# wang-xinyu/tensorrtx

Measured on AMD Instinct MI355X. Metric: images/sec @ batch=32 640x640 fp16 (yolov8n conv backbone + YoloLayer decode + NMS), higher is better.
Workload: dtype f16

## Files before the change

include/trtx_hip.h:

```cpp
#ifndef TRTX_HIP_H_
#define TRTX_HIP_H_

#include <stddef.h>
#include <stdint.h>

#ifdef __cplusplus
extern "C" {
#endif

#ifndef TRTX_NO_HIP_TYPES
struct ihipStream_t;
typedef struct ihipStream_t* trtx_stream_t;
#endif

#define TRTX_ABI_VERSION 1
#define TRTX_OK 0
#define TRTX_ERR_INVALID 1
#define TRTX_ERR_HIP 2
#define TRTX_ERR_WORKSPACE 3
#define TRTX_ERR_UNSUPPORTED 4
#define TRTX_ERR_NO_DEVICE 5
#define TRTX_ERR_IO 6
#define TRTX_ERR_STATE 7

// ... 138 lines not shown
#define TRTX_ACT_TANH 5
int32_t trtx_conv_packed_dims(int cout, int cin_pad, int kh, int kw, int32_t* cout_pad, int32_t* kpad, int32_t* bn);
int32_t trtx_conv_pack_weights_f16(const float* w_kcrs, int cout, int cin, int kh, int kw, int cin_pad,
                                   const float* ch_scale, uint16_t* packed);
int32_t trtx_op_conv2d_nhwc_f16(const void* in, int N, int H, int W, int Cin, int ld_in, const void* wpacked,
                                const float* bias, void* out, int Cout, int ld_out, int kh, int kw, int sh, int sw,
                                int ph, int pw, int act1, const void* residual, int ld_res, int act2,
                                trtx_stream_t stream);
int32_t trtx_op_conv2d_tactics(int N, int H, int W, int Cin, int ld_in, int Cout, int ld_out, int kh, int kw, int sh, int sw, int ph, int pw,
                               int has_residual, int ld_res, int32_t* out6, int32_t max_out);
int32_t trtx_op_conv_force_tactic(const int32_t* tactic6);
int32_t trtx_op_conv_stem_nchw_f16(const float* in, int N, int C, int H, int W, const float* w_taps_cout, const float* bias, void* out, int Cout,
                                   int ld_out, int k, int stride, int pad, int act, trtx_stream_t stream);
int32_t trtx_op_conv_stem_pair_f16(const float* in, int N, int C, int H, int W, const float* stem_w_taps_cout, const float* stem_bias, int stem_act,
                                   const void* conv_wpacked, const float* conv_bias, int conv_act, void* out, int ld_out, trtx_stream_t stream);
int32_t trtx_reorg_fold_weights(const float* w_kcrs, int cout, int cin, int kh, int kw, float* folded);
int32_t trtx_conv_packed_dims_f32(int cout, int cin_pad, int kh, int kw, int32_t* cout_pad, int32_t* kpad, int32_t* cink);
int32_t trtx_conv_pack_weights_f32(const float* w_kcrs, int cout, int cin, int kh, int kw, int cin_pad, const float* ch_scale, float* packed);
int32_t trtx_op_conv2d_nhwc_f32(const void* in, int N, int H, int W, int Cin, int ld_in, const void* wpacked, const float* bias, void* out, int Cout,
                                int ld_out, int kh, int kw, int sh, int sw, int ph, int pw, int act1, const void* residual, int ld_res, int act2,
                                const int32_t* tile4, trtx_stream_t stream);
int32_t trtx_op_conv2d_tactics_f32(int N, int H, int W, int Cin, int ld_in, int Cout, int ld_out, int kh, int kw, int sh, int sw, int ph, int pw,
                                   int has_residual, int ld_res, int32_t* out4, int32_t max_out);
int32_t trtx_conv_pack_weights_i8(const float* w_kcrs, int cout, int cin, int kh, int kw, const float* ch_scale, int8_t* packed, float* wscale_out,
                                  int32_t* cout_pad_out, int32_t* kpad_out);
int32_t trtx_op_conv2d_nhwc_i8(const void* in, int N, int H, int W, int Cin, int ld_in, const void* wpacked, const float* cscale, const float* bias, void* out,
                               int out_is_i8, float out_inv_scale, int Cout, int ld_out, int kh, int kw, int sh, int sw, int ph, int pw, int act1,
                               const void* residual, int res_is_i8, float res_scale, int ld_res, int act2, trtx_stream_t stream);
int32_t trtx_conv_pack_weights_grouped_f16(const float* w_kcrs, int cout, int cin_g, int kh, int kw, const float* ch_scale, uint16_t* packed,
                                           int32_t* kpad_out);
// ... 225 lines not shown
```

tensorrtx_amd/capi.py:

```python
import ctypes
import os

_HERE = os.path.dirname(os.path.abspath(__file__))
_LIB = None


class TrtxError(RuntimeError):
    def __init__(self, status, what):
        self.status = status
        msg = lib().trtx_status_string(status).decode() if _LIB is not None else "?"
        super().__init__(f"{what}: status {status} ({msg})")


def lib_path() -> str:
    return os.environ.get("TRTX_HIP_LIB") or os.path.join(_HERE, "lib", "libtrtx_hip.so")


def hip_runtimes_mapped():
    seen = []
    with open("/proc/self/maps") as f:
        for line in f:
            path = line.rsplit(" ", 1)[-1].strip()
            if "libamdhip64" in os.path.basename(path) and path not in seen:
                seen.append(path)
# ... 442 lines not shown
    return out


def conv_stem_pair_f16(x, stem_w_taps_cout, stem_bias, conv_wpacked, conv_bias, stem_act="silu", conv_act="silu", out=None, out_ld=None):
    import torch
    N, C, H, W = x.shape
    Hi, Wi = (H - 1) // 2 + 1, (W - 1) // 2 + 1
    Ho, Wo = (Hi - 1) // 2 + 1, (Wi - 1) // 2 + 1
    if out is None:
        out = torch.empty((N, Ho, Wo, 32), dtype=torch.float16, device=x.device)
    check(lib().trtx_op_conv_stem_pair_f16(_p(x), N, C, H, W, _p(stem_w_taps_cout), _p(stem_bias), ACT[stem_act], _p(conv_wpacked), _p(conv_bias),
                                           ACT[conv_act], _p(out), out_ld or out.shape[-1], _stream()), "trtx_op_conv_stem_pair_f16")
    return out


def pack_conv_weights_grouped_f16(w_kcrs, ch_scale=None):
    import numpy as np
    L = lib()
    w = np.ascontiguousarray(w_kcrs, dtype=np.float32)
    cout, cin_g, kh, kw = w.shape
    kp = ctypes.c_int32()
    check(L.trtx_conv_pack_weights_grouped_f16(w.ctypes.data_as(ctypes.c_void_p), cout, cin_g, kh, kw, None, None, ctypes.byref(kp)),
          "trtx_conv_pack_weights_grouped_f16 (dims)")
    packed = np.zeros((cout, kp.value), dtype=np.uint16)
    sc = None if ch_scale is None else np.ascontiguousarray(ch_scale, dtype=np.float32)
    check(L.trtx_conv_pack_weights_grouped_f16(w.ctypes.data_as(ctypes.c_void_p), cout, cin_g, kh, kw,
                                               sc.ctypes.data_as(ctypes.c_void_p) if sc is not None else None,
                                               packed.ctypes.data_as(ctypes.c_void_p), ctypes.byref(kp)), "trtx_conv_pack_weights_grouped_f16")
    return packed

# ... 200 lines not shown
```

tensorrtx_amd/csrc/kernels/kernels.h:

```cpp
#pragma once
#include <hip/hip_runtime.h>
#include <stddef.h>
#include <stdint.h>

namespace trtx {

enum Act : int { ACT_NONE = 0, ACT_RELU = 1, ACT_SIGMOID = 2, ACT_SILU = 3, ACT_LEAKY = 4, ACT_TANH = 5,
                 ACT_MISH = 6 ,
                 ACT_GELU_TANH = 7 ,
                 ACT_EXP = 8  };
enum DType : int { DT_F32 = 0, DT_F16 = 1, DT_I8 = 2 };
inline size_t dtype_size(int dt) { return dt == DT_F16 ? 2 : (dt == DT_I8 ? 1 : 4); }
enum EwOp : int { EW_SUM = 0, EW_PROD = 1, EW_MAX = 2, EW_MIN = 3, EW_SUB = 4, EW_DIV = 5, EW_POW = 6 };
enum PoolOp : int { POOL_MAX = 0, POOL_AVG = 1 };

enum Ws : int {
    WS_AUTO = 0,
    WS_OFF = 1,
    WS_ON = 2,
    WS_PATCH = 3,
    WS_F32_REGS = 5,
    WS_F32_ROLES = 6,
    WS_RES3 = 7,
    WS_RES1 = 8,
// ... 74 lines not shown
int32_t conv_ws_f16(const ConvArgs& a, hipStream_t s);
int32_t poison_lds(unsigned* device_word, hipStream_t s);
bool conv_stem_supported(const ConvArgs& a);
int32_t conv_stem_nchw_f32(const ConvArgs& a, hipStream_t s);
bool conv_stem_f32_supported(const ConvArgs& a);
int32_t conv_stem_nchw_f32_out_f32(const ConvArgs& a, hipStream_t s);
constexpr int kStemMaxFrames = 64;
struct StemFrame {
    const void* src;
    int w, h;
    float d2s[6];
};
int32_t conv_stem_frames_f32(const ConvArgs& a, const StemFrame* frames, hipStream_t s);
bool conv_stem_pair_possible(const ConvArgs& stem, const ConvArgs& conv);
int32_t conv_stem_pair_f16(const ConvArgs& stem, const ConvArgs& conv, hipStream_t s);
int32_t conv_direct(const ConvArgs& a, int dtype, hipStream_t s);
bool conv_dw_supported(const ConvArgs& a);
bool psa_attention_supported(int kd, int hd);
int32_t psa_attention_f16(const void* qkv, int ld_qkv, void* out, int ld_out, void* vimg, int ld_v, int B, int heads, int N, int kd, int hd,
                          float scale, hipStream_t s);
bool area_attention_supported(int kd, int hd);
int32_t area_attention_f16(const void* qkv, int ld_qkv, void* out, int ld_out, void* vimg, int ld_v, int B, int heads, int N, int area, int kd,
                           int hd, float scale, hipStream_t s);
bool area_attention_split_supported(int kd, int hd);
int32_t area_attention_split_f16(const void* q, int ld_q, const void* k, int ld_k, const void* v, int ld_v, void* out, int ld_out, int B, int heads, int N,
                                 int area, int kd, int hd, float scale, hipStream_t s);
int32_t conv_dw(const ConvArgs& a, int dtype, hipStream_t s);
struct HgconvWeights {
    const float* w_ctx;
    const float* b_ctx;
// ... 67 lines not shown
```

tensorrtx_amd/csrc/ops_capi.cpp:

```cpp
#include <hip/hip_runtime.h>
#include <stdlib.h>
#include <string.h>

#include <vector>

#include "common.h"
#include "options.h"
#include "kernels/kernels.h"
#include "runtime/pack.h"

using namespace trtx;

extern "C" const char* trtx_status_string(int32_t s) {
    switch (s) {
        case TRTX_OK: return "ok";
        case TRTX_ERR_INVALID: return "invalid argument";
        case TRTX_ERR_HIP: return "HIP error";
        case TRTX_ERR_WORKSPACE: return "workspace too small";
        case TRTX_ERR_UNSUPPORTED: return "unsupported configuration";
        case TRTX_ERR_NO_DEVICE: return "no HIP device";
        case TRTX_ERR_IO: return "I/O or parse error";
        case TRTX_ERR_STATE: return "invalid call order";
        default: return "unknown status";
    }
// ... 120 lines not shown
    a.ld_out = ld_out;
    return conv_stem_nchw_f32(a, static_cast<hipStream_t>(stream));
}

extern "C" int32_t trtx_op_conv_stem_pair_f16(const float* in, int N, int C, int H, int W, const float* stem_w_taps_cout, const float* stem_bias, int stem_act,
                                              const void* conv_wpacked, const float* conv_bias, int conv_act, void* out, int ld_out, trtx_stream_t stream) {
    if (!in || !stem_w_taps_cout || !conv_wpacked || !out || N < 1 || C < 1 || H < 1 || W < 1) return TRTX_ERR_INVALID;
    const ConvArgs s = op_stem_args(in, N, C, H, W, stem_w_taps_cout, stem_bias, 16, 3, 2, 1, stem_act);
    ConvArgs c = op_conv_args(N, s.Ho, s.Wo, 16, 16, 32, ld_out, 3, 3, 2, 2, 1, 1, conv_act, 0, 0, 0);
    c.wgt = conv_wpacked;
    c.bias = conv_bias;
    c.out = out;
    return conv_stem_pair_f16(s, c, static_cast<hipStream_t>(stream));
}

extern "C" int32_t trtx_conv_pack_weights_grouped_f16(const float* w_kcrs, int cout, int cin_g, int kh, int kw, const float* ch_scale, uint16_t* packed,
                                                      int32_t* kpad_out) {
    if (!w_kcrs || cout < 1 || cin_g < 1 || kh < 1 || kw < 1) return TRTX_ERR_INVALID;
    const int kpad = (kh * kw * cin_g + 31) / 32 * 32;
    if (kpad_out) *kpad_out = kpad;
    if (packed) pack_conv_weights_grouped_f16(w_kcrs, cout, cin_g, kh, kw, kpad, ch_scale, packed);
    return TRTX_OK;
}

extern "C" int32_t trtx_op_conv2d_grouped_nhwc_f16(const void* in, int N, int H, int W, int Cin, int ld_in, const void* wpacked, const float* bias, void* out,
                                                   int Cout, int ld_out, int groups, int k, int pad, int act1, const void* residual, int ld_res, int act2,
                                                   trtx_stream_t stream) {
    if (N < 1 || H < 1 || W < 1 || Cin < 1 || Cout < 1 || groups < 1 || k < 1 || pad < 0 || H + 2 * pad < k || W + 2 * pad < k) return TRTX_ERR_INVALID;
    ConvArgs a{};
    a.in = in; a.wgt = wpacked; a.bias = bias; a.out = out; a.residual = residual;
// ... 210 lines not shown
```

tensorrtx_amd/csrc/options.cpp:

```cpp
#include "options.h"

#include <stdlib.h>

namespace trtx {
namespace {
const char* env(const char* name) { return getenv(name); }
int env_int(const char* name, int unset) {
    const char* v = env(name);
    return (v && *v) ? atoi(v) : unset;
}
bool env_is(const char* name, int value) {
    const char* v = env(name);
    return v && *v && atoi(v) == value;
}
bool env_set(const char* name) { return env(name) != nullptr; }
}

Options read_options() {
    Options o;
    o.tune = env_int("TRTX_TUNE", -1);
    o.tune_verbose = env_set("TRTX_TUNE_VERBOSE");
    o.tune_margin = env_int("TRTX_TUNE_MARGIN", -1);
    if (const char* v = env("TRTX_TACTIC_CACHE")) o.tactic_cache = v;
    o.graph = env_is("TRTX_GRAPH", 1);
    if (const char* v = env("TRTX_CALIB_REPORT")) o.calib_report = v;
    if (const char* v = env("TRTX_INT8_CLIP_LIMIT"); v && *v) o.int8_clip_limit = atof(v);
    o.lanes = env_int("TRTX_LANES", 0);
    o.group_convs = !env_is("TRTX_GROUP_CONVS", 0);
    o.fold_upsample = !env_is("TRTX_FOLD_UPSAMPLE", 0);
    o.stem_pair = !env_is("TRTX_STEM_PAIR", 0);
    o.ws = !env_set("TRTX_CONV_NOWS");
    o.wsk = !env_set("TRTX_CONV_NOWSK");
    o.gemm256 = !env_is("TRTX_GEMM256", 0);
    o.patch = !env_is("TRTX_CONV_PATCH", 0);
    o.res = env_int("TRTX_CONV_RES", 7);
    o.roles = !env_is("TRTX_CONV_ROLES", 0);
    o.f32_mfma = !env_set("TRTX_F32_DIRECT");
    o.conv_grouped = !env_is("TRTX_CONV_GROUPED", 0);
    o.area_attention = !env_is("TRTX_AREA_ATTENTION", 0);
    o.aattn_split = !env_is("TRTX_AATTN_SPLIT", 0);
    o.hgconv = !env_is("TRTX_HGCONV", 0);
    o.gated_add = !env_is("TRTX_GATED_ADD", 0);
    o.yolo5_head = !env_is("TRTX_YOLO5_HEAD", 0);
    o.yolo7_head = !env_is("TRTX_YOLO7_HEAD", 0);
    o.reorg_fold = !env_is("TRTX_REORG_FOLD", 0);
// ... 16 lines not shown
```

tensorrtx_amd/csrc/options.h:

```cpp
#pragma once
#include <string>

namespace trtx {

struct Options {
    int tune = -1;
    bool tune_verbose = false;
    int tune_margin = -1;
    std::string tactic_cache;
    bool graph = false;
    std::string calib_report;
    double int8_clip_limit = 1e-4;
    int lanes = 0;
    bool group_convs = true;
    bool fold_upsample = true;
    bool stem_pair = true;
    bool ws = true;
    bool wsk = true;
    bool gemm256 = true;
    bool patch = true;
    int res = 7;
    bool roles = true;
    bool f32_mfma = true;
    bool conv_grouped = true;
    bool area_attention = true;
    bool aattn_split = true;
    bool hgconv = true;
    bool gated_add = true;
    bool yolo9_head = true;
    bool yolo5_head = true;
    bool yolo7_head = true;
// ... 13 lines not shown
```

tensorrtx_amd/csrc/runtime/engine.cpp:

```cpp
#include "engine.h"

#include <stdlib.h>
#include <string.h>

#include <sstream>

#include "../common.h"
#include "../options.h"
#include "int8.h"
#include "plugin.h"

using namespace trtx;

trtx_engine::~trtx_engine() {
    int left = plugins_initialized;
    for (auto& op : plan.ops)
        if (op.kind == OP_PLUGIN && left-- > 0 && op.plugin->v.terminate) op.plugin->v.terminate(op.plugin->v.self);
    if (d_weights) (void)hipFree(d_weights);
}

trtx_context::~trtx_context() {
    for (hipStream_t st : lane_stream)
        if (st) {
            (void)hipStreamSynchronize(st);
// ... 92 lines not shown
    std::vector<char> lane_started(plan.num_lanes, 0);
    auto bail = [&](int32_t st) {
        (void)hipGetLastError();
        if (lanes)
            for (int l = 1; l < plan.num_lanes; ++l)
                if (lane_started[l] && hipEventRecord(c->lane_done[l], c->lane_stream[l]) == hipSuccess)
                    (void)hipStreamWaitEvent(user_stream, c->lane_done[l], 0);
        for (auto& ev : evs) (void)hipEventDestroy(ev);
        evs.clear();
        free_probes();
        return st;
    };
    if (lanes && hipEventRecord(c->start_event, user_stream) != hipSuccess) return bail(TRTX_ERR_HIP);
    ConvArgs pair_stem{};
    bool pair_pending = false;
    for (size_t k = 0; k < plan.ops.size(); ++k) {
        const POp& op = plan.ops[k];
        hipStream_t stream = user_stream;
        if (lanes) {
            if (op.lane > 0) {
                stream = c->lane_stream[op.lane];
                if (!lane_started[op.lane]) {
                    if (hipStreamWaitEvent(stream, c->start_event, 0) != hipSuccess) return bail(TRTX_ERR_HIP);
                    lane_started[op.lane] = 1;
                }
            }
            for (int d : op.wait_ops)
                if (hipStreamWaitEvent(stream, c->op_event[d], 0) != hipSuccess) return bail(TRTX_ERR_HIP);
        }
        const PTensor& t0 = plan.tensors[op.in.empty() ? op.out[0] : op.in[0]];
// ... 23 lines not shown
                    b.N = nb(to);
                    b.M = b.N * b.Ho * b.Wo;
                    if (conv_stem_pair_possible(a, b)) {
                        pair_stem = a;
                        pair_pending = true;
                        break;
                    }
                }
                if (op.stem_pair && pair_pending) {
                    pair_pending = false;
                    if (prof && probes[k].start && probes[k].stop) conv_set_launch_probe(&probes[k]);
                    st = conv_stem_pair_f16(pair_stem, a, stream);
                    conv_set_launch_probe(nullptr);
                    break;
                }
                if (op.kind == OP_DECONV)
                    st = deconv_direct(a, op.dtype, stream);
                else if (op.stem && c->frames)
                    st = a.f32 ? TRTX_ERR_UNSUPPORTED : conv_stem_frames_f32(a, c->frames, stream);
                else if (op.stem)
                    st = a.f32 ? conv_stem_nchw_f32_out_f32(a, stream) : conv_stem_nchw_f32(a, stream);
                else if (op.igemm) {
                    if (prof && probes[k].start && probes[k].stop) conv_set_launch_probe(&probes[k]);
                    st = a.f32 ? conv_igemm_f32(a, stream) : conv_igemm_f16(a, stream);
                    conv_set_launch_probe(nullptr);
                } else if (op.dw)
                    st = conv_dw(a, op.dtype, stream);
                else if (op.grouped)
                    st = conv_grouped(a, stream);
                else
// ... 655 lines not shown
```

tensorrtx_amd/csrc/runtime/plan.cpp:

```cpp
#include "plan.h"

#include <sstream>

namespace trtx {

const char* op_kind_name(int k) {
    static const char* n[] = {"conv",     "deconv",    "pool",      "resize",     "ew_nhwc", "act_nhwc", "scale_nhwc",
                              "copy_nhwc", "reduce_hw", "to_nhwc",   "to_linear",  "gather",  "scatter",  "ew_lin",
                              "act_lin",  "scale_lin", "softmax",   "matmul",     "reduce_lin", "plugin", "copy_lin", "yolo_head",
                              "pool_chain", "depth_to_space", "roi_align", "conv_chain", "conv_group", "attention",
                              "yolo_task_head", "yolo5_head", "yolo9_head", "yolo7_head", "hgconv", "gated_add", "attention_split"};
    return (k >= 0 && k <= OP_ATTENTION_SPLIT) ? n[k] : "?";
}

std::string Plan::describe_json() const {
    std::ostringstream o;
    double flops = 0, bytes = 0;
    int n_conv = 0, n_igemm = 0;
    for (const auto& op : ops) {
        flops += op.flops;
        bytes += op.bytes;
        if (op.kind == OP_CONV) {
            ++n_conv;
            n_igemm += op.igemm ? 1 : 0;
        }
        n_conv += (int)op.group.size();
        n_igemm += (int)op.group.size();
    }
    o << "{\"fp16\":" << (fp16 ? "true" : "false") << ",\"max_batch\":" << max_batch << ",\"arena_bytes\":" << arena_bytes
      << ",\"weight_bytes\":" << weight_bytes << ",\"n_lanes\":" << num_lanes << ",\"n_ops\":" << ops.size() << ",\"n_conv\":" << n_conv
      << ",\"n_igemm\":" << n_igemm << ",\"flops_per_sample\":" << flops << ",\"bytes_per_sample\":" << bytes
      << ",\"ops\":[";
    for (size_t k = 0; k < ops.size(); ++k) {
        const POp& op = ops[k];
        o << (k ? "," : "") << "{\"kind\":\"" << op_kind_name(op.kind) << "\",\"name\":\"";
        for (char c : op.name) o << ((c == '"' || c == '\\' || (unsigned char)c < 0x20) ? ' ' : c);
        o << "\",\"flops\":" << op.flops << ",\"bytes\":" << op.bytes;
        auto conv_fields = [&](const POp& op) {
            const ConvArgs& a = op.conv;
            o << ",\"igemm\":" << (op.igemm ? "true" : "false") << ",\"stem\":" << (op.stem ? "true" : "false") << (op.stem_pair ? ",\"stem_pair\":true" : "") << ",\"cin\":" << (a.in_i8 ? 2 * a.Cin : a.Cin) << ",\"cout\":" << a.Cout
              << ",\"k\":[" << a.kh << "," << a.kw << "],\"stride\":[" << a.stride_h << "," << a.stride_w << "],\"hw_in\":["
              << a.H << "," << a.W << "],\"hw_out\":[" << a.Ho << "," << a.Wo << "],\"act1\":" << a.act1
              << ",\"act2\":" << a.act2 << ",\"alpha1\":" << a.alpha1 << ",\"alpha2\":" << a.alpha2 << ",\"up_c\":" << a.up_C << ",\"residual\":" << (op.in.size() > 1 ? "true" : "false")
              << ",\"bn_folded\":" << (op.scale_layer >= 0 ? "true" : "false") << ",\"ld_in\":" << a.ld_in
              << ",\"ld_out\":" << a.ld_out << ",\"i8\":[" << a.in_i8 << "," << a.out_i8 << "," << a.res_i8 << "],\"nmul\":" << (op.stem ? 1 : tensors[op.in[0]].nmul) << ",\"nfix\":"
              << (op.stem ? 0 : tensors[op.in[0]].nfix);
            if (op.dw) o << ",\"dw\":true";
            if (op.grouped) o << ",\"grouped\":true";
            if (op.cout_real) o << ",\"cout_real\":" << op.cout_real;
            if (op.reorg_cin) o << ",\"reorg_cin\":" << op.reorg_cin;
        };
        if (op.kind == OP_CONV || op.kind == OP_DECONV) conv_fields(op);
        if (op.kind == OP_ACT_NHWC || op.kind == OP_ACT_LIN) o << ",\"act\":" << op.i[0];
        if (op.kind == OP_ATTENTION) o << ",\"heads\":" << op.i[0] << ",\"n\":" << op.i[1] << ",\"kd\":" << op.i[2] << ",\"hd\":" << op.i[3];
        if (op.kind == OP_ATTENTION && op.i[4] > 0) o << ",\"area\":" << op.i[4] << ",\"kernel\":\"mfma\"";
// ... 75 lines not shown
```

tensorrtx_amd/csrc/runtime/plan.h:

```cpp
#pragma once
#include <memory>
#include <string>
#include <vector>

#include "../kernels/kernels.h"
#include "graph.h"
#include "plugin.h"

namespace trtx {

enum Layout : int { LAY_LINEAR = 0, LAY_NHWC = 1 };
enum StorageKind : int { ST_ARENA = 0, ST_WEIGHTS = 1, ST_BINDING = 2 };

enum OpKind : int {
    OP_CONV = 0,
    OP_DECONV,
    OP_POOL,
    OP_RESIZE,
    OP_EW_NHWC,
    OP_ACT_NHWC,
    OP_SCALE_NHWC,
    OP_COPY_NHWC,
    OP_REDUCE_HW,
    OP_TO_NHWC,
// ... 56 lines not shown
    int binding = -1;
    int first_use = 1 << 30, last_use = -1;
};
inline size_t align256(size_t v) { return (v + 255) / 256 * 256; }

struct POp {
    int kind = 0;
    std::string name;
    std::vector<int> in, out;
    std::vector<int> extra_in;
    int dtype = DT_F32;
    ConvArgs conv{};
    bool igemm = false;
    bool stem = false;
    bool stem_pair = false;
    bool from_deconv = false;
    bool dw = false;
    bool grouped = false;
    int reorg_cin = 0;
    int cout_real = 0;
    std::vector<POp> group;
    int src_layer = -1;
    int scale_layer = -1;
    size_t w_off = 0, b_off = 0, s_off = 0;
    int i[12] = {0};
    float f[4] = {0};
    std::vector<int> iv;
    std::vector<float> fv;
    StridedView view{};
    long off0 = 0;
// ... 39 lines not shown
```

tensorrtx_amd/csrc/runtime/plan_passes.cpp:

```cpp
#include "plan_passes.h"

#include <algorithm>

namespace trtx {
namespace {

bool fail(std::string* err, const std::string& m) {
    *err = m;
    return false;
}

size_t tensor_bytes(const Plan& plan, const PTensor& t) {
    const size_t es = dtype_size(t.dtype);
    if (t.layout == LAY_NHWC) {
        const size_t n = (t.nfix ? (size_t)t.nfix : (size_t)plan.max_batch) * (size_t)t.nmul;
        return n * t.H * t.W * (size_t)t.Calloc * es;
    }
    return (t.batched ? (size_t)plan.max_batch : 1) * (size_t)t.dims.volume() * es;
}

bool choose_conv_kernel(const Plan& plan, const PassInputs& e, POp& op) {
    ConvArgs& a = op.conv;
    const PTensor& ti = plan.tensors[op.in[0]];
    const PTensor& to = plan.tensors[op.out[0]];
// ... 639 lines not shown
            shared = touches(plan.ops[j]);
            for (const POp& m : plan.ops[j].group) shared = shared || touches(m);
        }
        if (shared) continue;
        ConvArgs a = st.conv, b = cv.conv;
        const PTensor& t_in = plan.tensors[st.in[0]];
        a.N = plan.explicit_batch ? (int)t_in.dims.d[0] : plan.max_batch;
        a.M = a.N * a.Ho * a.Wo;
        b.N = (mid.nfix ? mid.nfix : plan.max_batch) * mid.nmul;
        b.M = b.N * b.Ho * b.Wo;
        if (!conv_stem_pair_possible(a, b)) continue;
        cv.stem_pair = true;
    }
}

void assign_lanes(Plan& plan, const PassInputs& e, const std::vector<std::vector<int>>& deps) {
    const int nops = (int)plan.ops.size();
    int max_lanes = e.max_aux_streams >= 0 ? 1 + e.max_aux_streams : 4;
    if (e.opt.lanes > 0) max_lanes = std::max(1, std::min(16, e.opt.lanes));
    std::vector<int> tail(max_lanes, -1);
    plan.num_lanes = 1;
    for (int k = 0; k < nops; ++k) {
        int lane = -1;
        for (int d : deps[k])
            if (tail[plan.ops[d].lane] == d && (lane < 0 || d > tail[lane])) lane = plan.ops[d].lane;
        if (lane < 0 && deps[k].empty()) lane = 0;
        if (lane < 0) {
            for (int l = 0; l < max_lanes && lane < 0; ++l)
                if (tail[l] < 0) lane = l;
        }
// ... 23 lines not shown
    const int nops = (int)plan.ops.size();
    auto before = [&](int a, int b) { return a == b || anc.has(a, b); };
    std::vector<std::vector<int>> touch(plan.storages.size());
    for (int k = 0; k < nops; ++k) {
        const POp& op = plan.ops[k];
        auto mark = [&](int t) {
            const int st = plan.tensors[t].storage;
            Storage& s = plan.storages[st];
            s.first_use = std::min(s.first_use, k);
            s.last_use = std::max(s.last_use, k);
            if (touch[st].empty() || touch[st].back() != k) touch[st].push_back(k);
        };
        for (int t : op.in) mark(t);
        for (int t : op.extra_in) mark(t);
        for (int t : op.out) mark(t);
    }
    std::vector<std::pair<int, int>> ws_storage;
    for (int k = 0; k < nops; ++k) {
        const int kind = plan.ops[k].kind;
        if ((kind != OP_PLUGIN && kind != OP_YOLO_HEAD && kind != OP_YOLO_TASK_HEAD && kind != OP_YOLO5_HEAD && kind != OP_YOLO9_HEAD && kind != OP_YOLO7_HEAD && kind != OP_HGCONV) || plan.ops[k].ws_bytes == 0) continue;
        Storage s;
        s.kind = ST_ARENA;
        s.bytes = plan.ops[k].ws_bytes;
        s.first_use = s.last_use = k;
        ws_storage.push_back({k, (int)plan.storages.size()});
        plan.storages.push_back(s);
        touch.push_back({k});
    }
    auto ordered = [&](int sa, int sb) {
        for (int x : touch[sa])
// ... 31 lines not shown
    for (auto& w : ws_storage) plan.ops[w.first].ws_off = plan.storages[w.second].offset;
}

}

bool finalize_plan(Plan& plan, const PassInputs& e, std::string* err) {
    resolve_view_geometry(plan);
    fold_upsample(plan, e);
    assign_int8_served(plan, e);
    assign_storages(plan);
    if (!select_conv_kernels(plan, e, err) || !configure_plugins(plan, err)) return false;
    chain_sppf_pools(plan, e);
    chain_spp_parallel_pools(plan, e);
    group_convs(plan, e);
    mark_stem_pair(plan, e);
    const std::vector<std::vector<int>> deps = op_dependencies(plan);
    assign_lanes(plan, e, deps);
    plan_arena(plan, ancestors(plan, deps, true));
    return true;
}

}
```

Before: 38910.

## Fuse consecutive 16-channel 3x3 bottleneck convs into one tiled LDS kernel

```diff
diff --git a/include/trtx_hip.h b/include/trtx_hip.h
--- a/include/trtx_hip.h
+++ b/include/trtx_hip.h
@@ -176,6 +176,12 @@
                                    int ld_out, int k, int stride, int pad, int act, trtx_stream_t stream);
 int32_t trtx_op_conv_stem_pair_f16(const float* in, int N, int C, int H, int W, const float* stem_w_taps_cout, const float* stem_bias, int stem_act,
                                    const void* conv_wpacked, const float* conv_bias, int conv_act, void* out, int ld_out, trtx_stream_t stream);
+int32_t trtx_op_conv_bneck_pair_f16(const void* in, int N, int H, int W, int ld_in, int in_coff, const void* w1_packed, const float* bias1, int act1,
+                                    const void* w2_packed, const float* bias2, int act2, int shortcut, int act_after, void* out, int ld_out,
+                                    trtx_stream_t stream);
+int32_t trtx_op_conv_bneck_pair_or_two_f16(const void* in, int N, int H, int W, int ld_in, int in_coff, const void* w1_packed, const float* bias1, int act1,
+                                           const void* w2_packed, const float* bias2, int act2, int shortcut, int act_after, void* mid, void* out,
+                                           int ld_out, trtx_stream_t stream);
 int32_t trtx_reorg_fold_weights(const float* w_kcrs, int cout, int cin, int kh, int kw, float* folded);
 int32_t trtx_conv_packed_dims_f32(int cout, int cin_pad, int kh, int kw, int32_t* cout_pad, int32_t* kpad, int32_t* cink);
 int32_t trtx_conv_pack_weights_f32(const float* w_kcrs, int cout, int cin, int kh, int kw, int cin_pad, const float* ch_scale, float* packed);
diff --git a/tensorrtx_amd/capi.py b/tensorrtx_amd/capi.py
--- a/tensorrtx_amd/capi.py
+++ b/tensorrtx_amd/capi.py
@@ -480,6 +480,22 @@
     return out
 
 
+def conv_bneck_pair_f16(x, w1_packed, bias1, w2_packed, bias2, act1="silu", act2="silu", shortcut=True, act_after="none", out=None, out_ld=None, in_coff=None,
+                        mid=None):
+    import torch
+    N, H, W, C = x.shape
+    assert x.dtype == torch.float16 and x.stride(3) == 1 and (C == 16 if in_coff is None else in_coff + 16 <= C)
+    if out is None:
+        out = torch.empty((N, H, W, 16), dtype=torch.float16, device=x.device)
+    head = (_p(x), N, H, W, x.stride(2), in_coff or 0, _p(w1_packed), _p(bias1), ACT[act1], _p(w2_packed), _p(bias2), ACT[act2], 1 if shortcut else 0, ACT[act_after])
+    if mid is None:
+        check(lib().trtx_op_conv_bneck_pair_f16(*head, _p(out), out_ld or out.shape[-1], _stream()), "trtx_op_conv_bneck_pair_f16")
+    else:
+        assert mid.dtype == torch.float16 and mid.is_contiguous() and tuple(mid.shape) == (N, H, W, 16)
+        check(lib().trtx_op_conv_bneck_pair_or_two_f16(*head, _p(mid), _p(out), out_ld or out.shape[-1], _stream()), "trtx_op_conv_bneck_pair_or_two_f16")
+    return out
+
+
 def pack_conv_weights_grouped_f16(w_kcrs, ch_scale=None):
     import numpy as np
     L = lib()
diff --git a/tensorrtx_amd/csrc/kernels/bneck_pair_index.h b/tensorrtx_amd/csrc/kernels/bneck_pair_index.h
--- /dev/null
+++ b/tensorrtx_amd/csrc/kernels/bneck_pair_index.h
@@ -0,0 +1,88 @@
+#pragma once
+
+#if defined(__HIPCC__)
+#define TRTX_HD __host__ __device__ __forceinline__
+#else
+#define TRTX_HD inline
+#endif
+
+namespace trtx {
+namespace bneckidx {
+
+constexpr int kTH = 8, kTW = 16;
+constexpr int kRH = kTH + 2, kRW = kTW + 2;
+constexpr int kPH = kTH + 4, kPW = kTW + 4;
+constexpr int kRegionLin = (kRH - 1) * kPW + kRW;
+constexpr int kGroups = (kRegionLin + 15) / 16;
+constexpr int kPatchPixels = kPH * kPW;
+constexpr int kPatchChunks = 2 * kPatchPixels;
+constexpr int kFetch = (kPatchChunks + 255) / 256;
+constexpr int kPatchPlane = (kPatchPixels * 16 + 255) / 256 * 256;
+constexpr int kPatchBytes = 2 * kPatchPlane;
+constexpr int kImagePlane = (kRH * kPW * 16 + 255) / 256 * 256;
+constexpr int kImageBytes = 2 * kImagePlane;
+constexpr int kLdsBytes = 2 * kPatchBytes + kImageBytes;
+constexpr int kTaps = 9, kSteps = 5;
+static_assert(kPatchPixels % 8 == 0, "patch chunks are staged in runs of 8 pixels per plane");
+
+struct Tile {
+    int n, y0, x0;
+};
+TRTX_HD Tile tile_of(int tile, int tiles_x, int tiles_y) {
+    Tile t;
+    const int tx = tile % tiles_x;
+    const int rest = tile / tiles_x;
+    t.x0 = tx * kTW;
+    t.y0 = (rest % tiles_y) * kTH;
+    t.n = rest / tiles_y;
+    return t;
+}
+TRTX_HD int run_length(int total, int grid) { return (total + grid - 1) / grid; }
+TRTX_HD int run_first(int wg, int total, int grid) { return wg * run_length(total, grid); }
+
+struct PatchChunk {
+    int py, px, plane;
+};
+TRTX_HD PatchChunk patch_chunk(int c) {
+    const int j = c & 15;
+    const int pix = (c >> 4) * 8 + (j & 7);
+    PatchChunk p;
+    p.plane = j >> 3;
+    p.py = pix / kPW;
+    p.px = pix - p.py * kPW;
+    return p;
+}
+TRTX_HD int patch_offset(int py, int px, int plane) { return plane * kPatchPlane + (py * kPW + px) * 16; }
+TRTX_HD int image_offset(int ry, int rx, int ch) { return (ch >> 3) * kImagePlane + (ry * kPW + rx) * 16 + (ch & 7) * 2; }
+
+struct RegionPixel {
+    int ry, rx;
+    bool live;
+};
+TRTX_HD RegionPixel region_pixel(int group, int lane) {
+    const int e = group * 16 + (lane & 15);
+    const int ee = e < kRegionLin ? e : e - 16;
+    RegionPixel r;
+    r.ry = ee / kPW;
+    r.rx = ee - r.ry * kPW;
+    r.live = e < kRegionLin && r.rx < kRW;
+    return r;
+}
+TRTX_HD int step_tap(int kt, int lane) { return 2 * kt + ((lane >> 4) >> 1); }
+TRTX_HD int step_chunk(int lane) { return (lane >> 4) & 1; }
+TRTX_HD int frag1_offset(int ry, int rx, int tap, int chunk) {
+    const int r = tap / 3, q = tap - r * 3;
+    return patch_offset(ry + r, rx + q, chunk);
+}
+TRTX_HD int frag2_offset(int oy, int ox, int tap, int chunk) {
+    const int r = tap / 3, q = tap - r * 3;
+    return image_offset(oy + r, ox + q, chunk * 8);
+}
+TRTX_HD int lane_channel(int g) { return 8 * (g & 1) + 4 * (g >> 1); }
+TRTX_HD int weight_row_channel(int a) { return lane_channel(a >> 2) + (a & 3); }
+TRTX_HD int store_row(int wave, int lane) { return 2 * wave + (lane >> 5); }
+TRTX_HD int store_channel(int lane) { return 8 * ((lane >> 4) & 1); }
+TRTX_HD int shortcut_offset(int wave, int lane) { return patch_offset(store_row(wave, lane) + 2, (lane & 15) + 2, (lane >> 4) & 1); }
+
+}
+}
diff --git a/tensorrtx_amd/csrc/kernels/conv_bneck_pair.hip b/tensorrtx_amd/csrc/kernels/conv_bneck_pair.hip
--- /dev/null
+++ b/tensorrtx_amd/csrc/kernels/conv_bneck_pair.hip
@@ -0,0 +1,232 @@
+#include <hip/hip_fp16.h>
+#include <hip/hip_runtime.h>
+#include <stdint.h>
+
+#include "../common.h"
+#include "act.h"
+#include "bneck_pair_index.h"
+#include "kernels.h"
+#include "launch.h"
+
+namespace trtx {
+namespace {
+
+namespace bx = bneckidx;
+
+typedef unsigned uintx4 __attribute__((ext_vector_type(4)));
+typedef unsigned uintx2 __attribute__((ext_vector_type(2)));
+
+static_assert(bx::kLdsBytes <= 32 * 1024, "at least four workgroups per CU beside other contexts' workgroups");
+
+__device__ __forceinline__ unsigned bneck_pack_h2(_Float16 lo, _Float16 hi) {
+    typedef _Float16 half2v __attribute__((ext_vector_type(2)));
+    return __builtin_bit_cast(unsigned, half2v{lo, hi});
+}
+
+__device__ __forceinline__ _Float16 bneck_act1(float x, int act) {
+    if (act == ACT_SILU) return round_to_half(x * __builtin_amdgcn_rcpf(1.0f + __expf(-x)));
+    if (act == ACT_RELU) return round_to_half(x > 0.f ? x : 0.f);
+    return round_to_half(x);
+}
+
+__global__ __launch_bounds__(256) void conv_bneck_pair_kernel(const ConvArgs pa, const ConvArgs pb, int tiles_x, int tiles_y, int total_tiles) {
+    extern __shared__ __attribute__((aligned(256))) char s_lds[];
+    char* const s_img = s_lds + 2 * bx::kPatchBytes;
+    const int tid = threadIdx.x;
+    const int lane = tid & 63;
+    const int wave = __builtin_amdgcn_readfirstlane(tid >> 6);
+    const int grp = lane >> 4, col = lane & 15;
+
+    half8 wa[bx::kSteps], wb[bx::kSteps];
+    {
+        const _Float16* __restrict__ w0 = static_cast<const _Float16*>(pa.wgt);
+        const _Float16* __restrict__ w1 = static_cast<const _Float16*>(pb.wgt);
+        const int row = bx::weight_row_channel(col);
+#pragma unroll
+        for (int kt = 0; kt < bx::kSteps; ++kt) {
+            wa[kt] = *reinterpret_cast<const half8*>(w0 + (size_t)row * pa.Kpad + kt * 32 + grp * 8);
+            wb[kt] = *reinterpret_cast<const half8*>(w1 + (size_t)row * pb.Kpad + kt * 32 + grp * 8);
+        }
+    }
+    const int ch4 = bx::lane_channel(grp);
+    float4 ba = make_float4(0.f, 0.f, 0.f, 0.f), bb = ba;
+    if (pa.bias) ba = *reinterpret_cast<const float4*>(pa.bias + ch4);
+    if (pb.bias) bb = *reinterpret_cast<const float4*>(pb.bias + ch4);
+    const _Float16* __restrict__ in = static_cast<const _Float16*>(pa.in);
+    _Float16* __restrict__ out = static_cast<_Float16*>(pb.out);
+    const bool shortcut = pb.residual != nullptr, relu2 = pb.act2 != ACT_NONE;
+
+    uintx4 stage[bx::kFetch];
+    auto fetch = [&](int tile) {
+        const bx::Tile t = bx::tile_of(tile, tiles_x, tiles_y);
+#pragma unroll
+        for (int f = 0; f < bx::kFetch; ++f) {
+            const int c = tid + f * 256;
+            stage[f] = uintx4{0u, 0u, 0u, 0u};
+            if (c < bx::kPatchChunks) {
+                const bx::PatchChunk pc = bx::patch_chunk(c);
+                const int y = t.y0 - 2 + pc.py, x = t.x0 - 2 + pc.px;
+                if ((unsigned)y < (unsigned)pa.H && (unsigned)x < (unsigned)pa.W)
+                    stage[f] = *reinterpret_cast<const uintx4*>(in + (((size_t)t.n * pa.H + y) * pa.W + x) * pa.ld_in + pc.plane * 8);
+            }
+        }
+    };
+    auto land = [&](char* patch) {
+#pragma unroll
+        for (int f = 0; f < bx::kFetch; ++f) {
+            const int c = tid + f * 256;
+            if (c < bx::kPatchChunks) {
+                const bx::PatchChunk pc = bx::patch_chunk(c);
+                *reinterpret_cast<uintx4*>(patch + bx::patch_offset(pc.py, pc.px, pc.plane)) = stage[f];
+            }
+        }
+    };
+
+    const int per = bx::run_length(total_tiles, (int)gridDim.x);
+    const int first = bx::run_first((int)blockIdx.x, total_tiles, (int)gridDim.x);
+    const int last = first + per < total_tiles ? first + per : total_tiles;
+    if (first < last) fetch(first);
+    int buf = 0;
+    for (int tile = first; tile < last; ++tile, buf ^= 1) {
+        const bx::Tile t = bx::tile_of(tile, tiles_x, tiles_y);
+        char* const s_patch = s_lds + buf * bx::kPatchBytes;
+        land(s_patch);
+        __syncthreads();
+#pragma nounroll
+        for (int gi = wave; gi < bx::kGroups; gi += 4) {
+            const bx::RegionPixel rp = bx::region_pixel(gi, lane);
+            floatx4 acc = floatx4{0.f, 0.f, 0.f, 0.f};
+#pragma unroll
+            for (int kt = 0; kt < bx::kSteps; ++kt) {
+                const int tap = bx::step_tap(kt, lane);
+                half8 xf = half8{0, 0, 0, 0, 0, 0, 0, 0};
+                if (tap < bx::kTaps) xf = *reinterpret_cast<const half8*>(s_patch + bx::frag1_offset(rp.ry, rp.rx, tap, bx::step_chunk(lane)));
+                acc = __builtin_amdgcn_mfma_f32_16x16x32_f16(wa[kt], xf, acc, 0, 0, 0);
+            }
+            float x[4] = {acc[0], acc[1], acc[2], acc[3]};
+            if (pa.bias) {
+                x[0] += ba.x; x[1] += ba.y; x[2] += ba.z; x[3] += ba.w;
+            }
+            half4 o;
+#pragma unroll
+            for (int e = 0; e < 4; ++e) o[e] = bneck_act1(x[e], pa.act1);
+            const int iy = t.y0 - 1 + rp.ry, ix = t.x0 - 1 + rp.rx;
+            if ((unsigned)iy >= (unsigned)pa.Ho || (unsigned)ix >= (unsigned)pa.Wo) o = half4{0, 0, 0, 0};
+            if (rp.live) *reinterpret_cast<half4*>(s_img + bx::image_offset(rp.ry, rp.rx, ch4)) = o;
+        }
+        __syncthreads();
+        if (tile + 1 < last) fetch(tile + 1);
+        floatx4 acc[2] = {floatx4{0.f, 0.f, 0.f, 0.f}, floatx4{0.f, 0.f, 0.f, 0.f}};
+#pragma unroll
+        for (int kt = 0; kt < bx::kSteps; ++kt) {
+            const int tap = bx::step_tap(kt, lane);
+            half8 xf[2];
+#pragma unroll
+            for (int i = 0; i < 2; ++i) {
+                xf[i] = half8{0, 0, 0, 0, 0, 0, 0, 0};
+                if (tap < bx::kTaps) xf[i] = *reinterpret_cast<const half8*>(s_img + bx::frag2_offset(2 * wave + i, col, tap, bx::step_chunk(lane)));
+            }
+#pragma unroll
+            for (int i = 0; i < 2; ++i) acc[i] = __builtin_amdgcn_mfma_f32_16x16x32_f16(wb[kt], xf[i], acc[i], 0, 0, 0);
+        }
+        unsigned pk[2][2];
+#pragma unroll
+        for (int i = 0; i < 2; ++i) {
+            float x[4] = {acc[i][0], acc[i][1], acc[i][2], acc[i][3]};
+            if (pb.bias) {
+                x[0] += bb.x; x[1] += bb.y; x[2] += bb.z; x[3] += bb.w;
+            }
+            _Float16 h[4];
+#pragma unroll
+            for (int e = 0; e < 4; ++e) h[e] = bneck_act1(x[e], pb.act1);
+            pk[i][0] = bneck_pack_h2(h[0], h[1]);
+            pk[i][1] = bneck_pack_h2(h[2], h[3]);
+        }
+        const uintx2 s0 = __builtin_amdgcn_permlane32_swap(pk[0][0], pk[1][0], false, false);
+        const uintx2 s1 = __builtin_amdgcn_permlane32_swap(pk[0][1], pk[1][1], false, false);
+        const uintx4 q = {s0[0], s1[0], s0[1], s1[1]};
+        half8 v = __builtin_bit_cast(half8, q);
+        if (shortcut || relu2) {
+            half8 rv = half8{0, 0, 0, 0, 0, 0, 0, 0};
+            if (shortcut) rv = *reinterpret_cast<const half8*>(s_patch + bx::shortcut_offset(wave, lane));
+            if (!relu2) {
+#pragma unroll
+                for (int e = 0; e < 8; ++e) v[e] = round_to_half((float)v[e] + (float)rv[e]);
+            } else {
+#pragma unroll
+                for (int e = 0; e < 8; ++e) {
+                    const float s = (float)v[e] + (float)rv[e];
+                    v[e] = round_to_half(s > 0.f ? s : 0.f);
+                }
+            }
+        }
+        const int ho = t.y0 + bx::store_row(wave, lane), wo = t.x0 + col;
+        if (ho < pb.Ho && wo < pb.Wo) {
+            const size_t m = ((size_t)t.n * pb.Ho + ho) * pb.Wo + wo;
+            *reinterpret_cast<half8*>(out + m * pb.ld_out + bx::store_channel(lane)) = v;
+        }
+    }
+}
+
+bool bneck_layer_ok(const ConvArgs& c) {
+    const bool fast_act = c.act1 == ACT_SILU || c.act1 == ACT_RELU || c.act1 == ACT_NONE;
+    return !c.f32 && !c.in_i8 && !c.out_i8 && !c.res_i8 && !c.up_C && fast_act && !c.scalar_out && c.groups == 1 && c.dil_h == 1 && c.dil_w == 1 && c.Cin == 16 &&
+           c.CinK == 16 && c.bk == 32 && c.Kpad == 160 && c.Cout == 16 && c.Cout_pad == 16 && c.kh == 3 && c.kw == 3 && c.stride_h == 1 && c.stride_w == 1 &&
+           c.pad_h == 1 && c.pad_w == 1 && c.N >= 1 && c.H >= 1 && c.W >= 1 && c.Ho == c.H && c.Wo == c.W && (reinterpret_cast<uintptr_t>(c.wgt) & 15) == 0 &&
+           (reinterpret_cast<uintptr_t>(c.bias) & 15) == 0;
+}
+
+}
+
+bool conv_bneck_pair_possible(const ConvArgs& a, const ConvArgs& b) {
+    const bool first_ok = bneck_layer_ok(a) && !a.residual && a.act2 == ACT_NONE && a.ld_in % 8 == 0 && a.ld_in >= 16 &&
+                          (reinterpret_cast<uintptr_t>(a.in) & 15) == 0;
+    const bool second_ok = bneck_layer_ok(b) && (b.act2 == ACT_NONE || (b.act2 == ACT_RELU && b.residual)) && b.ld_out % 8 == 0 && b.ld_out >= 16 &&
+                           (reinterpret_cast<uintptr_t>(b.out) & 15) == 0;
+    const bool chained = b.N == a.N && b.H == a.Ho && b.W == a.Wo;
+    const bool shortcut_ok = !b.residual || !a.in || reinterpret_cast<uintptr_t>(b.residual) < 4096 || (b.residual == a.in && b.ld_res == a.ld_in);
+    bool apart = true;
+    if (a.in && b.out && first_ok && second_ok && chained) {
+        const intptr_t pin = reinterpret_cast<intptr_t>(a.in), pout = reinterpret_cast<intptr_t>(b.out);
+        const intptr_t pixels = (intptr_t)a.N * a.H * a.W;
+        const intptr_t in_bytes = ((pixels - 1) * a.ld_in + 16) * 2, out_bytes = ((pixels - 1) * b.ld_out + 16) * 2;
+        const intptr_t d = pout > pin ? pout - pin : pin - pout;
+        const bool disjoint = pin + in_bytes <= pout || pout + out_bytes <= pin;
+        const bool slices = a.ld_in == b.ld_out && d >= 32 && d + 32 <= (intptr_t)a.ld_in * 2;
+        apart = disjoint || slices;
+    }
+    return first_ok && second_ok && chained && shortcut_ok && apart;
+}
+
+int32_t conv_bneck_pair_or_two_f16(const ConvArgs& a, const ConvArgs& b, hipStream_t stream) {
+    if (conv_bneck_pair_possible(a, b) && a.in && a.wgt && b.wgt && b.out) return conv_bneck_pair_f16(a, b, stream);
+    if (!a.out || b.in != a.out) return TRTX_ERR_INVALID;
+    const int32_t st = conv_igemm_f16(a, stream);
+    return st != TRTX_OK ? st : conv_igemm_f16(b, stream);
+}
+
+int32_t conv_bneck_pair_f16(const ConvArgs& a, const ConvArgs& b, hipStream_t stream) {
+    if (!conv_bneck_pair_possible(a, b) || !a.in || !a.wgt || !b.wgt || !b.out || (b.residual && b.residual != a.in)) return TRTX_ERR_UNSUPPORTED;
+    namespace bx = bneckidx;
+    const int tiles_x = (b.Wo + bx::kTW - 1) / bx::kTW, tiles_y = (b.Ho + bx::kTH - 1) / bx::kTH;
+    const long total_l = (long)b.N * tiles_x * tiles_y;
+    if (total_l > 0x7fffffffL - 65536) return TRTX_ERR_UNSUPPORTED;
+    const int total = (int)total_l;
+    static thread_local int resident[2] = {-1, 0};
+    int dev = 0;
+    if (hipGetDevice(&dev) != hipSuccess) dev = 0;
+    if (resident[0] != dev || resident[1] <= 0) {
+        int per_cu = 0, cus = 0;
+        if (hipOccupancyMaxActiveBlocksPerMultiprocessor(&per_cu, conv_bneck_pair_kernel, 256, bx::kLdsBytes) != hipSuccess || per_cu < 1) per_cu = 1;
+        if (hipDeviceGetAttribute(&cus, hipDeviceAttributeMultiprocessorCount, dev) != hipSuccess || cus < 1) cus = 256;
+        (void)hipGetLastError();
+        resident[0] = dev;
+        resident[1] = per_cu * cus;
+    }
+    const int most = total < resident[1] ? total : resident[1];
+    const int grid = (total + bx::run_length(total, most) - 1) / bx::run_length(total, most);
+    TRTX_LAUNCH(conv_bneck_pair_kernel, dim3((unsigned)grid), dim3(256), bx::kLdsBytes, stream, a, b, tiles_x, tiles_y, total);
+    return check_launch("conv_bneck_pair_f16");
+}
+
+}
diff --git a/tensorrtx_amd/csrc/kernels/kernels.h b/tensorrtx_amd/csrc/kernels/kernels.h
--- a/tensorrtx_amd/csrc/kernels/kernels.h
+++ b/tensorrtx_amd/csrc/kernels/kernels.h
@@ -112,6 +112,9 @@
 int32_t conv_stem_frames_f32(const ConvArgs& a, const StemFrame* frames, hipStream_t s);
 bool conv_stem_pair_possible(const ConvArgs& stem, const ConvArgs& conv);
 int32_t conv_stem_pair_f16(const ConvArgs& stem, const ConvArgs& conv, hipStream_t s);
+bool conv_bneck_pair_possible(const ConvArgs& first, const ConvArgs& second);
+int32_t conv_bneck_pair_f16(const ConvArgs& first, const ConvArgs& second, hipStream_t s);
+int32_t conv_bneck_pair_or_two_f16(const ConvArgs& first, const ConvArgs& second, hipStream_t s);
 int32_t conv_direct(const ConvArgs& a, int dtype, hipStream_t s);
 bool conv_dw_supported(const ConvArgs& a);
 bool psa_attention_supported(int kd, int hd);
diff --git a/tensorrtx_amd/csrc/ops_capi.cpp b/tensorrtx_amd/csrc/ops_capi.cpp
--- a/tensorrtx_amd/csrc/ops_capi.cpp
+++ b/tensorrtx_amd/csrc/ops_capi.cpp
@@ -158,6 +158,39 @@
     return conv_stem_pair_f16(s, c, static_cast<hipStream_t>(stream));
 }
 
+static int32_t op_bneck_pair(const void* in, int N, int H, int W, int ld_in, int in_coff, const void* w1_packed, const float* bias1, int act1, const void* w2_packed,
+                             const float* bias2, int act2, int shortcut, int act_after, void* mid, void* out, int ld_out, bool or_two, trtx_stream_t stream) {
+    if (!in || !w1_packed || !w2_packed || !out || N < 1 || H < 1 || W < 1 || ld_in < 16 || ld_in % 8 || in_coff < 0 || in_coff % 8 || in_coff + 16 > ld_in ||
+        ld_out < 16 || ld_out % 8 || (or_two && !mid))
+        return TRTX_ERR_INVALID;
+    ConvArgs a = op_conv_args(N, H, W, 16, ld_in, 16, 16, 3, 3, 1, 1, 1, 1, act1, 0, 0, 0);
+    ConvArgs b = op_conv_args(N, H, W, 16, 16, 16, ld_out, 3, 3, 1, 1, 1, 1, act2, shortcut ? 1 : 0, shortcut ? ld_in : 0, act_after);
+    a.in = static_cast<const uint16_t*>(in) + in_coff;
+    a.wgt = w1_packed;
+    a.bias = bias1;
+    a.out = mid;
+    b.in = mid;
+    b.wgt = w2_packed;
+    b.bias = bias2;
+    b.out = out;
+    b.residual = shortcut ? a.in : nullptr;
+    if (or_two) return conv_bneck_pair_or_two_f16(a, b, static_cast<hipStream_t>(stream));
+    if (!conv_bneck_pair_possible(a, b)) return TRTX_ERR_INVALID;
+    return conv_bneck_pair_f16(a, b, static_cast<hipStream_t>(stream));
+}
+
+extern "C" int32_t trtx_op_conv_bneck_pair_f16(const void* in, int N, int H, int W, int ld_in, int in_coff, const void* w1_packed, const float* bias1, int act1,
+                                               const void* w2_packed, const float* bias2, int act2, int shortcut, int act_after, void* out, int ld_out,
+                                               trtx_stream_t stream) {
+    return op_bneck_pair(in, N, H, W, ld_in, in_coff, w1_packed, bias1, act1, w2_packed, bias2, act2, shortcut, act_after, nullptr, out, ld_out, false, stream);
+}
+
+extern "C" int32_t trtx_op_conv_bneck_pair_or_two_f16(const void* in, int N, int H, int W, int ld_in, int in_coff, const void* w1_packed, const float* bias1, int act1,
+                                                      const void* w2_packed, const float* bias2, int act2, int shortcut, int act_after, void* mid, void* out,
+                                                      int ld_out, trtx_stream_t stream) {
+    return op_bneck_pair(in, N, H, W, ld_in, in_coff, w1_packed, bias1, act1, w2_packed, bias2, act2, shortcut, act_after, mid, out, ld_out, true, stream);
+}
+
 extern "C" int32_t trtx_conv_pack_weights_grouped_f16(const float* w_kcrs, int cout, int cin_g, int kh, int kw, const float* ch_scale, uint16_t* packed,
                                                       int32_t* kpad_out) {
     if (!w_kcrs || cout < 1 || cin_g < 1 || kh < 1 || kw < 1) return TRTX_ERR_INVALID;
diff --git a/tensorrtx_amd/csrc/options.cpp b/tensorrtx_amd/csrc/options.cpp
--- a/tensorrtx_amd/csrc/options.cpp
+++ b/tensorrtx_amd/csrc/options.cpp
@@ -29,6 +29,7 @@
     o.group_convs = !env_is("TRTX_GROUP_CONVS", 0);
     o.fold_upsample = !env_is("TRTX_FOLD_UPSAMPLE", 0);
     o.stem_pair = !env_is("TRTX_STEM_PAIR", 0);
+    o.bneck_pair = !env_is("TRTX_BNECK_PAIR", 0);
     o.ws = !env_set("TRTX_CONV_NOWS");
     o.wsk = !env_set("TRTX_CONV_NOWSK");
     o.gemm256 = !env_is("TRTX_GEMM256", 0);
diff --git a/tensorrtx_amd/csrc/options.h b/tensorrtx_amd/csrc/options.h
--- a/tensorrtx_amd/csrc/options.h
+++ b/tensorrtx_amd/csrc/options.h
@@ -15,6 +15,7 @@
     bool group_convs = true;
     bool fold_upsample = true;
     bool stem_pair = true;
+    bool bneck_pair = true;
     bool ws = true;
     bool wsk = true;
     bool gemm256 = true;
diff --git a/tensorrtx_amd/csrc/runtime/engine.cpp b/tensorrtx_amd/csrc/runtime/engine.cpp
--- a/tensorrtx_amd/csrc/runtime/engine.cpp
+++ b/tensorrtx_amd/csrc/runtime/engine.cpp
@@ -130,6 +130,11 @@
     if (lanes && hipEventRecord(c->start_event, user_stream) != hipSuccess) return bail(TRTX_ERR_HIP);
     ConvArgs pair_stem{};
     bool pair_pending = false;
+    auto defers_to_next = [&](size_t k) {
+        if (c->observer || c->tuning || k + 1 >= plan.ops.size()) return false;
+        const POp &o = plan.ops[k], &nx = plan.ops[k + 1];
+        return nx.bneck_pair && nx.kind == OP_CONV && o.kind == OP_CONV && o.igemm && nx.lane == o.lane && nx.in[0] == o.out[0];
+    };
     for (size_t k = 0; k < plan.ops.size(); ++k) {
         const POp& op = plan.ops[k];
         hipStream_t stream = user_stream;
@@ -183,6 +188,21 @@
                     conv_set_launch_probe(nullptr);
                     break;
                 }
+                if (defers_to_next(k)) break;
+                if (op.bneck_pair && k > 0 && defers_to_next(k - 1)) {
+                    const POp& fo = plan.ops[k - 1];
+                    ConvArgs f = fo.conv;
+                    f.in = R.ptr(fo.in[0]);
+                    f.out = R.ptr(fo.out[0]);
+                    f.wgt = W + fo.w_off;
+                    f.bias = reinterpret_cast<const float*>(W + fo.b_off);
+                    f.N = nb(plan.tensors[fo.in[0]]);
+                    f.M = f.N * f.Ho * f.Wo;
+                    if (prof && probes[k].start && probes[k].stop) conv_set_launch_probe(&probes[k]);
+                    st = conv_bneck_pair_or_two_f16(f, a, stream);
+                    conv_set_launch_probe(nullptr);
+                    break;
+                }
                 if (op.kind == OP_DECONV)
                     st = deconv_direct(a, op.dtype, stream);
                 else if (op.stem && c->frames)
diff --git a/tensorrtx_amd/csrc/runtime/plan.cpp b/tensorrtx_amd/csrc/runtime/plan.cpp
--- a/tensorrtx_amd/csrc/runtime/plan.cpp
+++ b/tensorrtx_amd/csrc/runtime/plan.cpp
@@ -38,7 +38,8 @@
         o << "\",\"flops\":" << op.flops << ",\"bytes\":" << op.bytes;
         auto conv_fields = [&](const POp& op) {
             const ConvArgs& a = op.conv;
-            o << ",\"igemm\":" << (op.igemm ? "true" : "false") << ",\"stem\":" << (op.stem ? "true" : "false") << (op.stem_pair ? ",\"stem_pair\":true" : "") << ",\"cin\":" << (a.in_i8 ? 2 * a.Cin : a.Cin) << ",\"cout\":" << a.Cout
+            o << ",\"igemm\":" << (op.igemm ? "true" : "false") << ",\"stem\":" << (op.stem ? "true" : "false") << (op.stem_pair ? ",\"stem_pair\":true" : "")
+              << (op.bneck_pair ? ",\"bneck_pair\":true" : "") << ",\"cin\":" << (a.in_i8 ? 2 * a.Cin : a.Cin) << ",\"cout\":" << a.Cout
               << ",\"k\":[" << a.kh << "," << a.kw << "],\"stride\":[" << a.stride_h << "," << a.stride_w << "],\"hw_in\":["
               << a.H << "," << a.W << "],\"hw_out\":[" << a.Ho << "," << a.Wo << "],\"act1\":" << a.act1
               << ",\"act2\":" << a.act2 << ",\"alpha1\":" << a.alpha1 << ",\"alpha2\":" << a.alpha2 << ",\"up_c\":" << a.up_C << ",\"residual\":" << (op.in.size() > 1 ? "true" : "false")
diff --git a/tensorrtx_amd/csrc/runtime/plan.h b/tensorrtx_amd/csrc/runtime/plan.h
--- a/tensorrtx_amd/csrc/runtime/plan.h
+++ b/tensorrtx_amd/csrc/runtime/plan.h
@@ -94,6 +94,7 @@
     bool igemm = false;
     bool stem = false;
     bool stem_pair = false;
+    bool bneck_pair = false;
     bool from_deconv = false;
     bool dw = false;
     bool grouped = false;
diff --git a/tensorrtx_amd/csrc/runtime/plan_passes.cpp b/tensorrtx_amd/csrc/runtime/plan_passes.cpp
--- a/tensorrtx_amd/csrc/runtime/plan_passes.cpp
+++ b/tensorrtx_amd/csrc/runtime/plan_passes.cpp
@@ -677,6 +677,45 @@
     }
 }
 
+void mark_bneck_pair(Plan& plan, const PassInputs& e) {
+    if (!e.opt.bneck_pair || e.dt != DT_F16 || e.int8 || CalibrationLowering::active()) return;
+    const int n = (int)plan.ops.size();
+    auto plain = [](const POp& op) { return op.kind == OP_CONV && op.igemm && !op.stem && !op.stem_pair && !op.bneck_pair && !op.from_deconv && op.extra_in.empty() && op.out.size() == 1; };
+    for (int k = 0; k + 1 < n; ++k) {
+        const POp& c0 = plan.ops[k];
+        POp& c1 = plan.ops[k + 1];
+        if (!plain(c0) || !plain(c1) || c0.in.size() != 1 || c1.in.empty() || c1.in.size() > 2 || c1.in[0] != c0.out[0]) continue;
+        if (c1.in.size() == 2 && c1.in[1] != c0.in[0]) continue;
+        const PTensor& mid = plan.tensors[c0.out[0]];
+        if (mid.parent >= 0 || mid.storage < 0 || plan.storages[mid.storage].kind != ST_ARENA || is_binding_tensor(plan, mid.id)) continue;
+        bool shared = false;
+        auto touches = [&](const POp& op) {
+            for (const std::vector<int>* v : {&op.in, &op.out, &op.extra_in})
+                for (int t : *v)
+                    if (plan.tensors[t].storage == mid.storage) return true;
+            return false;
+        };
+        for (int j = 0; j < n && !shared; ++j) {
+            if (j == k || j == k + 1) continue;
+            shared = touches(plan.ops[j]);
+            for (const POp& m : plan.ops[j].group) shared = shared || touches(m);
+        }
+        const PTensor &t_in = plan.tensors[c0.in[0]], &t_out = plan.tensors[c1.out[0]];
+        if (shared || t_in.storage == mid.storage || t_out.storage == mid.storage) continue;
+        if (t_in.layout != LAY_NHWC || t_out.layout != LAY_NHWC) continue;
+        if (t_in.storage == t_out.storage && t_in.rcoff < t_out.rcoff + std::max(t_out.C, 1) && t_out.rcoff < t_in.rcoff + std::max(t_in.C, 1)) continue;
+        ConvArgs a = c0.conv, b = c1.conv;
+        a.N = (t_in.nfix ? t_in.nfix : plan.max_batch) * t_in.nmul;
+        a.M = a.N * a.Ho * a.Wo;
+        b.N = (mid.nfix ? mid.nfix : plan.max_batch) * mid.nmul;
+        b.M = b.N * b.Ho * b.Wo;
+        b.residual = c1.in.size() > 1 ? reinterpret_cast<const void*>(1) : nullptr;
+        if (!conv_bneck_pair_possible(a, b)) continue;
+        c1.bneck_pair = true;
+        ++k;
+    }
+}
+
 void assign_lanes(Plan& plan, const PassInputs& e, const std::vector<std::vector<int>>& deps) {
     const int nops = (int)plan.ops.size();
     int max_lanes = e.max_aux_streams >= 0 ? 1 + e.max_aux_streams : 4;
@@ -730,6 +769,8 @@
         for (int t : op.in) mark(t);
         for (int t : op.extra_in) mark(t);
         for (int t : op.out) mark(t);
+        if (op.bneck_pair && k > 0)
+            for (int t : plan.ops[k - 1].in) mark(t);
     }
     std::vector<std::pair<int, int>> ws_storage;
     for (int k = 0; k < nops; ++k) {
@@ -791,8 +832,11 @@
     chain_spp_parallel_pools(plan, e);
     group_convs(plan, e);
     mark_stem_pair(plan, e);
+    mark_bneck_pair(plan, e);
     const std::vector<std::vector<int>> deps = op_dependencies(plan);
     assign_lanes(plan, e, deps);
+    for (size_t k = 1; k < plan.ops.size(); ++k)
+        if (plan.ops[k].bneck_pair && (plan.ops[k].lane != plan.ops[k - 1].lane || plan.ops[k - 1].signal)) plan.ops[k].bneck_pair = false;
     plan_arena(plan, ancestors(plan, deps, true));
     return true;
 }
```

Result: faster. 40500 (median of 6 runs) (+4.1%).
